# LeeBY68/Hier-SLAM

Measured on AMD Instinct MI355X. Metric: fwd+bwd renders/sec @1200x680, 500k Gaussians, 4-level tree; grad max-abs-err vs ref, higher is better.
Workload: dtype f32; 1 GPU; semantic fwd+bwd render, 1200x680, P=500000 slam Gaussians, K=26 semantic channels, dense upstream grads on colour/semantic/depth/median/opacity; P=500000, visible=480888, num_rendered=1136056, width=1200, height=680, K=26, parallelism=single GPU, keyframes_per_rank=1

## Files before the change

hier-slam_amd/csrc/hsr_render_fwd.hip:

```cpp

#include "hsr_tile_common.h"

#ifdef HSR_TRACE
__device__ unsigned long long g_hsr_trace_fwd[16384 * 8];
extern "C" int hsr_debug_read_trace_fwd(unsigned long long* host, int n)
{
    return (int)hipMemcpyFromSymbol(host, HIP_SYMBOL(g_hsr_trace_fwd), sizeof(unsigned long long) * (size_t)n);
}
#define TRF_NOW() clock64()
#define TRF_ADD(acc, t0) (acc) += (unsigned long long)(clock64() - (t0))
#else
#define TRF_NOW() 0ll
#define TRF_ADD(acc, t0) ((void)0)
#endif

namespace {

template <int W>
__device__ __forceinline__ void quad_fma_words(float (&s)[16], const float (&x)[4], float w)
{
    static_assert(W >= 1 && W <= 4, "1..4 words = 4..16 channels per block");
    if constexpr (W == 4) {
        asm("s_nop 1\n\t"
            "v_fmac_f32_dpp %0, %16, %20 quad_perm:[0,0,0,0] row_mask:0xf bank_mask:0xf\n\t"
            "v_fmac_f32_dpp %1, %16, %20 quad_perm:[1,1,1,1] row_mask:0xf bank_mask:0xf\n\t"
            "v_fmac_f32_dpp %2, %16, %20 quad_perm:[2,2,2,2] row_mask:0xf bank_mask:0xf\n\t"
            "v_fmac_f32_dpp %3, %16, %20 quad_perm:[3,3,3,3] row_mask:0xf bank_mask:0xf\n\t"
            "v_fmac_f32_dpp %4, %17, %20 quad_perm:[0,0,0,0] row_mask:0xf bank_mask:0xf\n\t"
            "v_fmac_f32_dpp %5, %17, %20 quad_perm:[1,1,1,1] row_mask:0xf bank_mask:0xf\n\t"
            "v_fmac_f32_dpp %6, %17, %20 quad_perm:[2,2,2,2] row_mask:0xf bank_mask:0xf\n\t"
            "v_fmac_f32_dpp %7, %17, %20 quad_perm:[3,3,3,3] row_mask:0xf bank_mask:0xf\n\t"
            "v_fmac_f32_dpp %8, %18, %20 quad_perm:[0,0,0,0] row_mask:0xf bank_mask:0xf\n\t"
            "v_fmac_f32_dpp %9, %18, %20 quad_perm:[1,1,1,1] row_mask:0xf bank_mask:0xf\n\t"
            "v_fmac_f32_dpp %10, %18, %20 quad_perm:[2,2,2,2] row_mask:0xf bank_mask:0xf\n\t"
            "v_fmac_f32_dpp %11, %18, %20 quad_perm:[3,3,3,3] row_mask:0xf bank_mask:0xf\n\t"
            "v_fmac_f32_dpp %12, %19, %20 quad_perm:[0,0,0,0] row_mask:0xf bank_mask:0xf\n\t"
            "v_fmac_f32_dpp %13, %19, %20 quad_perm:[1,1,1,1] row_mask:0xf bank_mask:0xf\n\t"
            "v_fmac_f32_dpp %14, %19, %20 quad_perm:[2,2,2,2] row_mask:0xf bank_mask:0xf\n\t"
            "v_fmac_f32_dpp %15, %19, %20 quad_perm:[3,3,3,3] row_mask:0xf bank_mask:0xf"
            : "+v"(s[0]), "+v"(s[1]), "+v"(s[2]), "+v"(s[3]), "+v"(s[4]), "+v"(s[5]), "+v"(s[6]), "+v"(s[7]), "+v"(s[8]), "+v"(s[9]), "+v"(s[10]), "+v"(s[11]), "+v"(s[12]), "+v"(s[13]), "+v"(s[14]), "+v"(s[15])
            : "v"(x[0]), "v"(x[1]), "v"(x[2]), "v"(x[3]), "v"(w));
    } else if constexpr (W == 3) {
        asm("s_nop 1\n\t"
            "v_fmac_f32_dpp %0, %12, %15 quad_perm:[0,0,0,0] row_mask:0xf bank_mask:0xf\n\t"
            "v_fmac_f32_dpp %1, %12, %15 quad_perm:[1,1,1,1] row_mask:0xf bank_mask:0xf\n\t"
            "v_fmac_f32_dpp %2, %12, %15 quad_perm:[2,2,2,2] row_mask:0xf bank_mask:0xf\n\t"
            "v_fmac_f32_dpp %3, %12, %15 quad_perm:[3,3,3,3] row_mask:0xf bank_mask:0xf\n\t"
            "v_fmac_f32_dpp %4, %13, %15 quad_perm:[0,0,0,0] row_mask:0xf bank_mask:0xf\n\t"
            "v_fmac_f32_dpp %5, %13, %15 quad_perm:[1,1,1,1] row_mask:0xf bank_mask:0xf\n\t"
            "v_fmac_f32_dpp %6, %13, %15 quad_perm:[2,2,2,2] row_mask:0xf bank_mask:0xf\n\t"
            "v_fmac_f32_dpp %7, %13, %15 quad_perm:[3,3,3,3] row_mask:0xf bank_mask:0xf\n\t"
            "v_fmac_f32_dpp %8, %14, %15 quad_perm:[0,0,0,0] row_mask:0xf bank_mask:0xf\n\t"
            "v_fmac_f32_dpp %9, %14, %15 quad_perm:[1,1,1,1] row_mask:0xf bank_mask:0xf\n\t"
            "v_fmac_f32_dpp %10, %14, %15 quad_perm:[2,2,2,2] row_mask:0xf bank_mask:0xf\n\t"
            "v_fmac_f32_dpp %11, %14, %15 quad_perm:[3,3,3,3] row_mask:0xf bank_mask:0xf"
            : "+v"(s[0]), "+v"(s[1]), "+v"(s[2]), "+v"(s[3]), "+v"(s[4]), "+v"(s[5]), "+v"(s[6]), "+v"(s[7]), "+v"(s[8]), "+v"(s[9]), "+v"(s[10]), "+v"(s[11])
            : "v"(x[0]), "v"(x[1]), "v"(x[2]), "v"(w));
    } else if constexpr (W == 2) {
        asm("s_nop 1\n\t"
            "v_fmac_f32_dpp %0, %8, %10 quad_perm:[0,0,0,0] row_mask:0xf bank_mask:0xf\n\t"
            "v_fmac_f32_dpp %1, %8, %10 quad_perm:[1,1,1,1] row_mask:0xf bank_mask:0xf\n\t"
            "v_fmac_f32_dpp %2, %8, %10 quad_perm:[2,2,2,2] row_mask:0xf bank_mask:0xf\n\t"
            "v_fmac_f32_dpp %3, %8, %10 quad_perm:[3,3,3,3] row_mask:0xf bank_mask:0xf\n\t"
            "v_fmac_f32_dpp %4, %9, %10 quad_perm:[0,0,0,0] row_mask:0xf bank_mask:0xf\n\t"
            "v_fmac_f32_dpp %5, %9, %10 quad_perm:[1,1,1,1] row_mask:0xf bank_mask:0xf\n\t"
            "v_fmac_f32_dpp %6, %9, %10 quad_perm:[2,2,2,2] row_mask:0xf bank_mask:0xf\n\t"
            "v_fmac_f32_dpp %7, %9, %10 quad_perm:[3,3,3,3] row_mask:0xf bank_mask:0xf"
            : "+v"(s[0]), "+v"(s[1]), "+v"(s[2]), "+v"(s[3]), "+v"(s[4]), "+v"(s[5]), "+v"(s[6]), "+v"(s[7])
            : "v"(x[0]), "v"(x[1]), "v"(w));
    } else {
        asm("s_nop 1\n\t"
            "v_fmac_f32_dpp %0, %4, %5 quad_perm:[0,0,0,0] row_mask:0xf bank_mask:0xf\n\t"
            "v_fmac_f32_dpp %1, %4, %5 quad_perm:[1,1,1,1] row_mask:0xf bank_mask:0xf\n\t"
            "v_fmac_f32_dpp %2, %4, %5 quad_perm:[2,2,2,2] row_mask:0xf bank_mask:0xf\n\t"
            "v_fmac_f32_dpp %3, %4, %5 quad_perm:[3,3,3,3] row_mask:0xf bank_mask:0xf"
            : "+v"(s[0]), "+v"(s[1]), "+v"(s[2]), "+v"(s[3])
            : "v"(x[0]), "v"(w));
    }
}

template <int KC, bool BASE, bool MASK, bool ALIGNED, bool PF = false>
__global__ void __launch_bounds__(256, KC <= 26 ? (KC == 16 ? 5 : 4) : (PF ? (KC <= 48 ? 4 : (KC <= 80 ? 3 : 2)) : 1)) render_fwd_kernel(RenderFwdArgs a, int c0)
{
    constexpr int BATCH = KC <= 32 ? (KC > 26 ? 200 : 240)
                                   : (KC <= 48 ? 152 : ((KC <= 64 || KC == 74) ? 144 : (KC <= 80 ? 136 : (KC <= 112 ? 144 : 128))));
    static_assert(KC <= 32 || PF, "batch sizes beyond 32 channels assume the touched rows (PF)");
    constexpr int RW = (KC + 2 + 3) & ~3;
    constexpr bool QS = PF && KC > 0;
    constexpr int NGF = QS ? RW / 16 : 0;
    constexpr int REM = QS ? (RW % 16) / 4 : 0;
    __shared__ float4 s_rec[BATCH * 2];
    __shared__ float4 s_row[BATCH * (RW / 4)];
    __shared__ uint8_t s_sublist[16 * HSR_SUB_LSTRIDE];
    __shared__ uint8_t s_subcnt[4][16];
    __shared__ int s_wdone[4];

    const int tile = hsr_block_tile(blockIdx.x, hsr_num_tiles(a.W, a.H));
    if (tile >= hsr_num_tiles(a.W, a.H)) return;
    const int t = threadIdx.x, wv = t >> 6;
    if (a.bin.base) {
        BinState bs;
        if (!hsr_bin_resolve(a.bin, *a.bin.R_dev, &bs)) {
            hsr_poison_tile(a, tile, t, BASE, c0, KC);
            return;
        }
        a.point_list = bs.vals;
        a.masks = bs.vals_unsorted;
    }
    const TileGeom tg = tile_geom_sub(tile, a.W, a.H, t);
    const bool inside = tg.inside;
    const size_t N = (size_t)a.W * a.H;
    float pfx = tg.pfx, pfy = tg.pfy;
    asm volatile("" : "+v"(pfx), "+v"(pfy));
    const float tile_x0 = (float)(tg.tx * HSR_TILE_X), tile_y0 = (float)(tg.ty * HSR_TILE_Y);

    unsigned long long tr_bar = 0, tr_stage = 0, tr_blend = 0, tr_iters = 0, tr_pub = 0;
    (void)tr_pub;
    const long long tr_t0 = TRF_NOW();
    long long tr_t1 = tr_t0;
    (void)tr_bar; (void)tr_stage; (void)tr_blend; (void)tr_iters; (void)tr_t0; (void)tr_t1;
    const uint2 range = a.ranges[tile];
    const int n = (int)(range.y - range.x);

    float T = 1.0f;
    uint32_t last_contributor = 0;
    float C0 = 0, C1 = 0, C2 = 0, Dd = 0, Mm = 0;
    uint32_t median_at = 0;
    float median_D = 15.0f;
    float S[KC > 0 ? KC : 1];
#pragma unroll
    for (int c = 0; c < (KC > 0 ? KC : 1); c++) S[c] = 0.f;
    bool done = !inside;

    int id_next = 0;
    float2 p_xy = {0, 0};
    float4 p_co = {0, 0, 0, 0};
    float p_r = 0, p_g = 0, p_b = 0, p_d = 0;
    float p_sem[(KC > 0 && !PF) ? KC : 1];
#pragma unroll
    for (int c = 0; c < ((KC > 0 && !PF) ? KC : 1); c++) p_sem[c] = 0.f;
    constexpr int NPF = PF ? (KC + 15) / 16 + 1 : 1;
    float pf_t[NPF];
#pragma unroll
    for (int c = 0; c < NPF; c++) pf_t[c] = 0.f;
    float pf_sink = 0.f;
    int id_cur = 0;

    auto fetch_id = [&](int start) -> int { return (int)a.point_list[range.x + min(max(start + t, 0), n - 1)]; };
    auto load_record = [&](int id_of) {
        const size_t id = (size_t)id_of;
        id_cur = id_of;
        {
            const float4* rec = a.rec + 4 * id;
            const float4 r0 = rec[0];
            p_co = rec[1];
            p_xy = make_float2(r0.x, r0.y);
            p_d = r0.z;
            if (BASE) {
                const float4 r2 = rec[2];
                p_r = r2.x; p_g = r2.y; p_b = r2.z;
            }
            if (KC > 0 && PF) {
                const float* row = a.semantics + id * (size_t)a.K + c0;
                const int last = min(KC, a.K - c0) - 1;
#pragma unroll
                for (int c = 0; c < NPF; c++) pf_t[c] = row[min(16 * c, last)];
            } else if (KC > 0) {
                if (ALIGNED) {
                    const float2* row = reinterpret_cast<const float2*>(a.semantics + id * (size_t)KC);
#pragma unroll
                    for (int q = 0; q < KC / 2; q++) {
                        const float2 v = row[q];
                        p_sem[PF ? 0 : 2 * q] = v.x;
                        p_sem[PF ? 0 : 2 * q + 1] = v.y;
                    }
                } else {
                    const float* row = a.semantics + id * (size_t)a.K + c0;
#pragma unroll
                    for (int c = 0; c < KC; c++) p_sem[PF ? 0 : c] = (c0 + c < a.K) ? row[c] : 0.f;
                }
            }
        }
    };
    if (n > 0) {
        const int id0 = fetch_id(0);
        id_next = fetch_id(BATCH);
        load_record(id0);
    }
    auto resolve_median = [&](int start) {
        if (BASE && median_at > (uint32_t)start) {
            const int j = (int)median_at - 1 - start;
            constexpr int c = KC + 1;
            constexpr int pos = (QS && c / 16 < NGF) ? (16 * (c / 16) + 4 * (c % 4) + (c % 16) / 4) : c;
            median_D = reinterpret_cast<const float*>(s_row)[j * RW + pos];
        }
    };


    for (int start = 0; start < n; start += BATCH) {
        const bool wave_done = __ballot(!done) == 0ull;
        if ((t & 63) == 0) s_wdone[wv] = wave_done;
        const long long tb0 = TRF_NOW();
        (void)tb0;
        __syncthreads();
        TRF_ADD(tr_bar, tb0);
        if (start == 0) tr_t1 = TRF_NOW();
        const long long ts0 = TRF_NOW();
        (void)ts0;
        if (s_wdone[0] & s_wdone[1] & s_wdone[2] & s_wdone[3]) break;
        const int cnt = min(BATCH, n - start);
        uint32_t mask16 = 0u;
        if (t < cnt) {
            mask16 = subblock_mask(p_xy.x, p_xy.y, p_co.x, p_co.y, p_co.z, p_co.w, tile_x0, tile_y0);
            a.masks[range.x + start + t] = mask16;
            s_rec[2 * t] = make_float4(p_xy.x, p_xy.y, (-0.5f * HSR_LOG2E) * p_co.x, -HSR_LOG2E * p_co.y);
            s_rec[2 * t + 1] = make_float4((-0.5f * HSR_LOG2E) * p_co.z, p_co.w, p_r, p_g);
            float4* row = &s_row[t * (RW / 4)];
            if (PF) {
#pragma unroll
                for (int c = 0; c < NPF; c++) pf_sink += pf_t[c];
                const float* grow = a.semantics + (size_t)id_cur * (size_t)a.K + c0;
                if (mask16 != 0u || t == 0)
#pragma unroll
                for (int g0 = 0; g0 < RW; g0 += 32) {
                    float rv[32];
#pragma unroll
                    for (int c = 0; c < 32; c++) {
                        const int ch = g0 + c;
                        if (ch < KC) {
                            if (ALIGNED) {
                                if ((c & 1) == 0) {
                                    const float2 v = reinterpret_cast<const float2*>(grow)[ch / 2];
                                    rv[c] = v.x;
                                    if (c + 1 < 32) rv[c + 1] = v.y;
                                }
                            } else {
                                rv[c] = (c0 + ch < a.K) ? grow[ch] : 0.f;
                            }
                        } else if (ch < RW) {
                            rv[c] = ch == KC ? p_b : (ch == KC + 1 ? p_d : 0.f);
                        }
                    }
#pragma unroll
                    for (int q = 0; q < 8; q++)
                        if (g0 / 4 + q < RW / 4) {
                            if (QS && g0 / 16 + q / 4 < NGF) {
                                const int b = 16 * (q / 4) + (q & 3);
                                row[g0 / 4 + q] = make_float4(rv[b], rv[b + 4], rv[b + 8], rv[b + 12]);
                            } else {
                                row[g0 / 4 + q] = make_float4(rv[4 * q], rv[4 * q + 1], rv[4 * q + 2], rv[4 * q + 3]);
                            }
                        }
                    asm volatile("" ::: "memory");
                }
            } else {
                float rv[RW];
#pragma unroll
                for (int c = 0; c < RW; c++) rv[c] = c < KC ? p_sem[(c < KC && !PF) ? c : 0] : (c == KC ? p_b : (c == KC + 1 ? p_d : 0.f));
#pragma unroll
                for (int q = 0; q < RW / 4; q++) {
                    if (QS && q / 4 < NGF) {
                        const int b = 16 * (q / 4) + (q & 3);
                        row[q] = make_float4(rv[b], rv[b + 4], rv[b + 8], rv[b + 12]);
                    } else {
                        row[q] = make_float4(rv[4 * q], rv[4 * q + 1], rv[4 * q + 2], rv[4 * q + 3]);
                    }
                }
            }
        }
        const long long tp0 = TRF_NOW();
        (void)tp0;
        publish_subblock_lists(mask16, t, s_sublist, s_subcnt);
        TRF_ADD(tr_pub, tp0);
        TRF_ADD(tr_stage, ts0);
        const long long tb1 = TRF_NOW();
        (void)tb1;
        __syncthreads();
        TRF_ADD(tr_bar, tb1);
        const long long tl0 = TRF_NOW();
        (void)tl0;
        {
            const int id_use = id_next;
            id_next = fetch_id(start + 2 * BATCH);
            load_record(id_use);
        }
        if (wave_done) continue;

        const int lane = t & 63, sb = wv * 4 + (lane >> 4);
        const int total = flatten_sublist(sb, lane, s_sublist, s_subcnt);
        const int m = __builtin_amdgcn_readfirstlane(max(max(__builtin_amdgcn_readlane(total, 0), __builtin_amdgcn_readlane(total, 16)),
                                                         max(__builtin_amdgcn_readlane(total, 32), __builtin_amdgcn_readlane(total, 48))));
        const uint8_t* list = s_sublist + sb * HSR_SUB_LSTRIDE;
        if (total == 0 && (lane & 15) == 0) s_sublist[sb * HSR_SUB_LSTRIDE] = 0;
        __builtin_amdgcn_fence(__ATOMIC_RELEASE, "wavefront");
        __builtin_amdgcn_wave_barrier();
        __builtin_amdgcn_fence(__ATOMIC_ACQUIRE, "wavefront");
        const int last = max(total - 1, 0);
        if constexpr (QS) {
            constexpr int NW = 4 * NGF + REM;
            constexpr int NCH = KC + (BASE ? 2 : 0);
            int j_next = (int)list[0];
            for (int k = 0; k < m; k++) {
                const int j = j_next;
                const bool valid = k < total;
                j_next = (int)list[min(k + 1, last)];
                const float4 g = s_rec[2 * j];
                const float4 h4 = s_rec[2 * j + 1];
                const float2 co = make_float2(h4.x, h4.y);
                const float dx = g.x - pfx, dy = g.y - pfy;
                const float power2 = fmaf(co.x, dy * dy, fmaf(g.w, dx * dy, g.z * (dx * dx)));
                const float alpha = fminf(0.99f, co.y * __builtin_amdgcn_exp2f(power2));
                bool contrib = valid && !done && power2 <= 0.0f && alpha >= 1.0f / 255.0f;
                const float test_T = T * (1.0f - alpha);
                if (contrib && test_T < 0.0001f) {
                    done = true;
                    contrib = false;
                }
                if (__ballot(contrib) == 0ull) continue;
                const float w = contrib ? alpha * T : 0.f;
                if (BASE) {
                    C0 = fmaf(h4.z, w, C0);
                    C1 = fmaf(h4.w, w, C1);
                    if (MASK) Mm += w;
                }
                const float* rowf = reinterpret_cast<const float*>(s_row) + j * RW;
                float fq[NW];
#pragma unroll
                for (int G = 0; G < NGF; G++) {
                    const float4 f = *reinterpret_cast<const float4*>(rowf + 16 * G + 4 * (lane & 3));
                    fq[4 * G] = f.x; fq[4 * G + 1] = f.y; fq[4 * G + 2] = f.z; fq[4 * G + 3] = f.w;
                }
#pragma unroll
                for (int mm = 0; mm < REM; mm++) fq[4 * NGF + mm] = rowf[16 * NGF + 4 * mm + (lane & 3)];
                float dummy = 0.f;
                auto acc = [&](int c) -> float& { return c < KC ? S[c < KC ? c : 0] : ((BASE && c == KC) ? C2 : ((BASE && c == KC + 1) ? Dd : dummy)); };
#pragma unroll
                for (int b = 0; b < (NCH + 15) / 16; b++) {
                    const int nw = min(4, (NCH - 16 * b + 3) / 4);
                    float sv[16], xv[4];
#pragma unroll
                    for (int i = 0; i < 16; i++) sv[i] = i < 4 * nw ? acc(16 * b + i) : 0.f;
#pragma unroll
                    for (int i = 0; i < 4; i++) xv[i] = i < nw ? fq[4 * b + i] : 0.f;
                    if (nw == 4) quad_fma_words<4>(sv, xv, w);
                    else if (nw == 3) quad_fma_words<3>(sv, xv, w);
                    else if (nw == 2) quad_fma_words<2>(sv, xv, w);
                    else quad_fma_words<1>(sv, xv, w);
#pragma unroll
                    for (int i = 0; i < 16; i++)
                        if (i < 4 * nw && 16 * b + i < NCH) acc(16 * b + i) = sv[i];
                }
                if (BASE) {
                    if (contrib && T > 0.5f && test_T < 0.5f) median_at = (uint32_t)(start + j + 1);
                }
                if (contrib) {
                    T = test_T;
                    last_contributor = (uint32_t)(start + j + 1);
                }
#ifdef HSR_TRACE
                tr_iters++;
#endif
            }
        } else {
            int j_next = (int)list[0];
            for (int k = 0; k < m; k++) {
                const int j = j_next;
                const bool valid = k < total;
                j_next = (int)list[min(k + 1, last)];
                const float4 g = s_rec[2 * j];
                const float4 h4 = s_rec[2 * j + 1];
                const float2 co = make_float2(h4.x, h4.y);
                const float dx = g.x - pfx, dy = g.y - pfy;
                const float power2 = fmaf(co.x, dy * dy, fmaf(g.w, dx * dy, g.z * (dx * dx)));
                const float alpha = fminf(0.99f, co.y * __builtin_amdgcn_exp2f(power2));
                bool contrib = valid && !done && power2 <= 0.0f && alpha >= 1.0f / 255.0f;
                const float test_T = T * (1.0f - alpha);
                if (contrib && test_T < 0.0001f) {
                    done = true;
                    contrib = false;
                }
                if (__ballot(contrib) == 0ull) continue;
                const float w = contrib ? alpha * T : 0.f;
                if (BASE) {
                    C0 = fmaf(h4.z, w, C0);
                    C1 = fmaf(h4.w, w, C1);
                    if (MASK) Mm += w;
                }
                {
                    const float4* row = &s_row[j * (RW / 4)];
#pragma unroll
                    for (int q = 0; q < RW / 4; q++) {
                        const float4 f = row[q];
                        const float fv[4] = {f.x, f.y, f.z, f.w};
#pragma unroll
                        for (int i = 0; i < 4; i++) {
                            const int c = 4 * q + i;
                            if (c < KC) S[c < KC ? c : 0] = fmaf(fv[i], w, S[c < KC ? c : 0]);
                            else if (BASE && c == KC) C2 = fmaf(fv[i], w, C2);
                            else if (BASE && c == KC + 1) {
                                Dd = fmaf(fv[i], w, Dd);
                                if (contrib && T > 0.5f && test_T < 0.5f) median_at = (uint32_t)(start + j + 1);
                            }
                        }
                    }
                }
                if (contrib) {
                    T = test_T;
                    last_contributor = (uint32_t)(start + j + 1);
                }
#ifdef HSR_TRACE
                tr_iters++;
#endif
            }
        }
        TRF_ADD(tr_blend, tl0);
        resolve_median(start);
        continue;
    }

    if (PF && pf_sink == 1.2345678e-30f) T = pf_sink;
#ifdef HSR_TRACE
    const long long tr_t2 = clock64();
#endif
    if (inside) {
        const size_t pix_id = (size_t)a.W * (size_t)(int)pfy + (size_t)(int)pfx;
        if (BASE) {
            a.final_T[pix_id] = T;
            a.n_contrib[pix_id] = last_contributor;
            a.median_pos[pix_id] = median_at;
            a.out_color[pix_id] = C0;
            a.out_color[N + pix_id] = C1;
            a.out_color[2 * N + pix_id] = C2;
            a.out_depth[pix_id] = Dd;
            a.out_median_depth[pix_id] = median_D;
            a.out_opacity[pix_id] = 1.0f - T;
            if (MASK) a.out_mask[pix_id] = Mm;
        }
        if (KC > 0) {
#pragma unroll
            for (int c = 0; c < KC; c++)
                if (c0 + c < a.K) a.out_semantic[(size_t)(c0 + c) * N + pix_id] = S[c];
        }
    }
#ifdef HSR_TRACE
    if ((t & 63) == 0) {
        const int wid = tile * 4 + wv;
        if (wid < 16384) {
            unsigned long long* o = g_hsr_trace_fwd + (size_t)wid * 8;
            o[0] = (unsigned long long)(clock64() - tr_t0);
            o[1] = (unsigned long long)(tr_t1 - tr_t0);
            o[2] = tr_bar; o[3] = tr_stage; o[4] = tr_blend;
            o[5] = (unsigned long long)(clock64() - tr_t2);
            o[6] = tr_iters;
            o[7] = tr_pub;
        }
    }
#endif
}

}

int hsr_launch_render_forward(const RenderFwdArgs& a, hipStream_t stream)
{
    const dim3 grid(hsr_tile_grid(hsr_num_tiles(a.W, a.H))), block(256);
    if (!a.semantic) {
        render_fwd_kernel<0, true, true, false><<<grid, block, 0, stream>>>(a, 0);
        return HSR_OK;
    }
    if (a.K >= 27 && a.K <= 128 && a.K != 74 && a.K != 102) {
        if (a.K <= 32) render_fwd_kernel<32, true, false, false, true><<<grid, block, 0, stream>>>(a, 0);
        else if (a.K <= 48) render_fwd_kernel<48, true, false, false, true><<<grid, block, 0, stream>>>(a, 0);
        else if (a.K <= 64) render_fwd_kernel<64, true, false, false, true><<<grid, block, 0, stream>>>(a, 0);
        else if (a.K <= 80) render_fwd_kernel<80, true, false, false, true><<<grid, block, 0, stream>>>(a, 0);
        else if (a.K <= 96) render_fwd_kernel<96, true, false, false, true><<<grid, block, 0, stream>>>(a, 0);
        else if (a.K <= 112) render_fwd_kernel<112, true, false, false, true><<<grid, block, 0, stream>>>(a, 0);
        else render_fwd_kernel<128, true, false, false, true><<<grid, block, 0, stream>>>(a, 0);
        return HSR_OK;
    }
    switch (a.K) {
    case 0: render_fwd_kernel<0, true, false, false><<<grid, block, 0, stream>>>(a, 0); return HSR_OK;
    case 16: render_fwd_kernel<16, true, false, true><<<grid, block, 0, stream>>>(a, 0); return HSR_OK;
    case 26: render_fwd_kernel<26, true, false, true><<<grid, block, 0, stream>>>(a, 0); return HSR_OK;
    case 74: render_fwd_kernel<74, true, false, true, true><<<grid, block, 0, stream>>>(a, 0); return HSR_OK;
    case 102: render_fwd_kernel<102, true, false, true, true><<<grid, block, 0, stream>>>(a, 0); return HSR_OK;
    default:
        render_fwd_kernel<32, true, false, false><<<grid, block, 0, stream>>>(a, 0);
        for (int c0 = 32; c0 < a.K; c0 += 32) render_fwd_kernel<32, false, false, false><<<grid, block, 0, stream>>>(a, c0);
        return HSR_OK;
    }
}
```

hier-slam_amd/csrc/hsr_tile_common.h:

```cpp
#pragma once
#include "hsr_common.h"

#define HSR_LOG2E 1.4426950408889634f

__host__ __device__ inline int hsr_num_tiles(int W, int H) { return ((W + HSR_TILE_X - 1) / HSR_TILE_X) * ((H + HSR_TILE_Y - 1) / HSR_TILE_Y); }
__host__ __device__ inline int hsr_tile_grid(int T) { return 8 * ((T + 7) / 8); }
__device__ __forceinline__ int hsr_block_tile(int b, int T) { return (b & 7) * ((T + 7) >> 3) + (b >> 3); }

__device__ __forceinline__ void hsr_poison_tile(const RenderFwdArgs& a, int tile, int t, bool base, int c0, int nsem)
{
    const int tiles_x = (a.W + HSR_TILE_X - 1) / HSR_TILE_X;
    const int px = (tile % tiles_x) * HSR_TILE_X + (t & 15), py = (tile / tiles_x) * HSR_TILE_Y + (t >> 4);
    if (px >= a.W || py >= a.H) return;
    const size_t N = (size_t)a.W * a.H, pix = (size_t)a.W * py + px;
    const float nan = __uint_as_float(0x7fc00000u);
    if (base) {
        a.out_color[pix] = nan; a.out_color[N + pix] = nan; a.out_color[2 * N + pix] = nan;
        a.out_depth[pix] = nan; a.out_median_depth[pix] = nan; a.out_opacity[pix] = nan;
        if (a.out_mask) a.out_mask[pix] = nan;
    }
    if (a.out_semantic)
        for (int c = c0; c < c0 + nsem && c < a.K; c++) a.out_semantic[(size_t)c * N + pix] = nan;
}

struct TileGeom {
    int tx, ty;
    int px, py;
    bool inside;
    float pfx, pfy;
    float qx0, qy0;
};

__device__ __forceinline__ TileGeom tile_geom(int tile, int W, int H, int t)
{
    TileGeom g;
    const int tiles_x = (W + HSR_TILE_X - 1) / HSR_TILE_X;
    g.tx = tile % tiles_x;
    g.ty = tile / tiles_x;
    const int wv = t >> 6, l = t & 63;
    const int qx = (wv & 1) * 8, qy = (wv >> 1) * 8;
    g.px = g.tx * HSR_TILE_X + qx + (l & 7);
    g.py = g.ty * HSR_TILE_Y + qy + (l >> 3);
    g.inside = g.px < W && g.py < H;
    g.pfx = (float)g.px;
    g.pfy = (float)g.py;
    g.qx0 = (float)(g.tx * HSR_TILE_X + qx);
    g.qy0 = (float)(g.ty * HSR_TILE_Y + qy);
    return g;
}

__device__ __forceinline__ void publish_quadrant_lists(uint32_t qmask, int t, uint8_t (*s_list)[256], uint8_t (*s_lcnt)[4])
{
    const int lane = t & 63, sw = t >> 6;
    const uint64_t lt = (1ull << lane) - 1ull;
#pragma unroll
    for (int q = 0; q < 4; q++) {
        const bool on = (qmask >> q) & 1u;
        const uint64_t m = __ballot(on);
        if (on) s_list[q][sw * 64 + __popcll(m & lt)] = (uint8_t)t;
        if (lane == 0) s_lcnt[q][sw] = (uint8_t)__popcll(m);
    }
}

__device__ __forceinline__ int build_flat_list(int wv, int lane, const uint8_t (*s_list)[256], const uint8_t (*s_lcnt)[4],
                                               uint8_t (*s_flat)[256])
{
    int total = 0;
#pragma unroll
    for (int seg = 0; seg < 4; seg++) {
        const int c = s_lcnt[wv][seg];
        if (lane < c) s_flat[wv][total + lane] = s_list[wv][seg * 64 + lane];
        total += c;
    }
    __builtin_amdgcn_wave_barrier();
    return total;
}

__device__ __forceinline__ TileGeom tile_geom_sub(int tile, int W, int H, int t)
{
    TileGeom g;
    const int tiles_x = (W + HSR_TILE_X - 1) / HSR_TILE_X;
    g.tx = tile % tiles_x;
    g.ty = tile / tiles_x;
    const int wv = t >> 6, l = t & 63, gq = l >> 4;
    const int qx = (wv & 1) * 8 + (gq & 1) * 4, qy = (wv >> 1) * 8 + (gq >> 1) * 4;
    g.px = g.tx * HSR_TILE_X + qx + (l & 3);
    g.py = g.ty * HSR_TILE_Y + qy + ((l >> 2) & 3);
    g.inside = g.px < W && g.py < H;
    g.pfx = (float)g.px;
    g.pfy = (float)g.py;
    g.qx0 = (float)(g.tx * HSR_TILE_X + qx);
    g.qy0 = (float)(g.ty * HSR_TILE_Y + qy);
    return g;
}

__device__ __forceinline__ uint32_t subblock_mask(float x, float y, float cx, float cy, float cz, float opacity, float tile_x0,
                                                  float tile_y0)
{
    const float t255 = 255.0f * opacity;
    if (!(t255 >= 1.0f)) return 0u;
    const float tau = 2.0f * __logf(t255) * 1.002f + 0.02f;
    const float det = cx * cz - cy * cy;
    if (!(det > 0.0f) || !(cx > 0.0f) || !(cz > 0.0f)) return 0xFFFFu;
    const float inv_det = 1.0f / det, inv_a = 1.0f / cx;
    const float hx = sqrtf(tau * cz * inv_det), hy = sqrtf(tau * cx * inv_det) * 1.001f + 0.02f;
    const float dyp = -(cy / cz) * hx;
    const float atau = cx * tau, nb = -cy;
    const float rx = x - tile_x0, ry = y - tile_y0;
    uint32_t m = 0u;
    float ry_hi = ry;
#pragma nounroll
    for (int r = 0; r < 4; r++, ry_hi -= 4.0f) {
        const float lo = fmaxf(ry_hi - 3.0f, -hy), hi = fminf(ry_hi, hy);
        const float dyu = __builtin_amdgcn_fmed3f(dyp, lo, hi), dyl = __builtin_amdgcn_fmed3f(-dyp, lo, hi);
        const float xmax = fmaf(nb, dyu, sqrtf(fmaxf(fmaf(-det * dyu, dyu, atau), 0.0f))) * inv_a + 0.02f;
        const float xmin = fmaf(nb, dyl, -sqrtf(fmaxf(fmaf(-det * dyl, dyl, atau), 0.0f))) * inv_a - 0.02f;
        uint32_t rb = 0u;
#pragma unroll
        for (int c = 0; c < 4; c++)
            rb |= (uint32_t)((rx - (4.0f * c + 3.0f)) <= xmax && (rx - 4.0f * c) >= xmin) << (4 * (c >> 1) + (c & 1));
        if (lo <= hi) m |= rb << (8 * (r >> 1) + 2 * (r & 1));
    }
    return m;
}

__device__ __forceinline__ uint32_t quadrant_bits(uint32_t mask)
{
    return (uint32_t)((mask & 0xFu) != 0u) | ((uint32_t)((mask & 0xF0u) != 0u) << 1) | ((uint32_t)((mask & 0xF00u) != 0u) << 2) |
           ((uint32_t)((mask & 0xF000u) != 0u) << 3);
}
__device__ __forceinline__ uint32_t quadrant_mask_exact(float x, float y, float cx, float cy, float cz, float opacity, float tile_x0,
                                                        float tile_y0)
{
    return quadrant_bits(subblock_mask(x, y, cx, cy, cz, opacity, tile_x0, tile_y0));
}

constexpr int HSR_SUB_LSTRIDE = 260;

__device__ __forceinline__ void publish_subblock_lists(uint32_t mask, int t, uint8_t* s_list, uint8_t (*s_lcnt)[16])
{
    const int lane = t & 63, sw = t >> 6;
    const uint64_t lt = (1ull << lane) - 1ull;
#pragma unroll
    for (int b = 0; b < 16; b++) {
        const bool on = (mask >> b) & 1u;
        const uint64_t m = __ballot(on);
        if (on) s_list[b * HSR_SUB_LSTRIDE + sw * 64 + __popcll(m & lt)] = (uint8_t)t;
        if (lane == 0) s_lcnt[sw][b] = (uint8_t)__popcll(m);
    }
}

__device__ __forceinline__ int flatten_sublist(int sb, int lane, uint8_t* s_list, const uint8_t (*s_lcnt)[16])
{
    const int l16 = lane & 15;
    uint8_t* list = s_list + sb * HSR_SUB_LSTRIDE;
    int total = s_lcnt[0][sb];
#pragma unroll
    for (int seg = 1; seg < 4; seg++) {
        const int c = s_lcnt[seg][sb];
        if (total != seg * 64) {
#pragma unroll
            for (int i = 0; i < 64; i += 16) {
                const bool mv = i + l16 < c;
                const uint8_t v = list[seg * 64 + i + l16];
                if (mv) list[total + i + l16] = v;
            }
        }
        total += c;
    }
    __builtin_amdgcn_wave_barrier();
    return total;
}

#define HSR_GROW_SEM0 16
__host__ __device__ inline int hsr_grow_stride(int K) { return 16 + 16 * ((K + 5 + 15) / 16); }
__host__ __device__ inline int hsr_grow_direct0(int K) { return HSR_GROW_SEM0 + K; }
__host__ __device__ inline int hsr_grow_nl0(int K) { return K + 5 < 9 ? K + 5 : 9; }
__host__ __device__ inline int hsr_grow_stride_l(int layout, int K)
{
    if (!layout) return hsr_grow_stride(K);
    const int R = K + 5 - hsr_grow_nl0(K);
    return 16 + 16 * ((R + 15) / 16);
}
__host__ __device__ inline int hsr_grow_col(int layout, int K, int ch)
{
    if (!layout) return HSR_GROW_SEM0 + ch;
    const int R = K + 5 - hsr_grow_nl0(K);
    return ch < R ? HSR_GROW_SEM0 + ch : 7 + (ch - R);
}
__host__ __device__ inline bool hsr_grow_compact_pays(int K) { return hsr_grow_stride_l(1, K) < hsr_grow_stride(K); }
```

Before: 1820 renders/s.

## Pad sub-block lists with a zero dummy slot to drop per-step bounds checks

For the non-prefetch forward path, each sub-block list is padded up to the wave-max length with an index pointing at a zeroed dummy record slot, so the blend loop no longer clamps indices or tests validity. Termination is folded into T itself (T set to zero on saturation or outside pixels), and a separate T_out keeps the true transmittance for output. Last-contributor and median indices are tracked as batch-relative integers and resolved once per batch rather than per step. This shortens the inner loop and removes branches, at the cost of an extra shared-memory slot, padding writes, and more delicate numerical bookkeeping for early termination.

```diff
diff --git a/hier-slam_amd/csrc/hsr_render_fwd.hip b/hier-slam_amd/csrc/hsr_render_fwd.hip
--- a/hier-slam_amd/csrc/hsr_render_fwd.hip
+++ b/hier-slam_amd/csrc/hsr_render_fwd.hip
@@ -89,8 +89,10 @@
     constexpr bool QS = PF && KC > 0;
     constexpr int NGF = QS ? RW / 16 : 0;
     constexpr int REM = QS ? (RW % 16) / 4 : 0;
-    __shared__ float4 s_rec[BATCH * 2];
-    __shared__ float4 s_row[BATCH * (RW / 4)];
+    constexpr int NSLOT = BATCH + (QS ? 0 : 1);
+    static_assert(NSLOT <= 256, "list entries are bytes");
+    __shared__ float4 s_rec[NSLOT * 2];
+    __shared__ float4 s_row[NSLOT * (RW / 4)];
     __shared__ uint8_t s_sublist[16 * HSR_SUB_LSTRIDE];
     __shared__ uint8_t s_subcnt[4][16];
     __shared__ int s_wdone[4];
@@ -122,7 +124,7 @@
     const uint2 range = a.ranges[tile];
     const int n = (int)(range.y - range.x);
 
-    float T = 1.0f;
+    float T = (QS || inside) ? 1.0f : 0.0f, T_out = 1.0f;
     uint32_t last_contributor = 0;
     float C0 = 0, C1 = 0, C2 = 0, Dd = 0, Mm = 0;
     uint32_t median_at = 0;
@@ -145,6 +147,11 @@
     for (int c = 0; c < NPF; c++) pf_t[c] = 0.f;
     float pf_sink = 0.f;
     int id_cur = 0;
+
+    if constexpr (!QS) {
+        if (t < 2) s_rec[2 * BATCH + t] = make_float4(0.f, 0.f, 0.f, 0.f);
+        if (t < RW / 4) s_row[BATCH * (RW / 4) + t] = make_float4(0.f, 0.f, 0.f, 0.f);
+    }
 
     auto fetch_id = [&](int start) -> int { return (int)a.point_list[range.x + min(max(start + t, 0), n - 1)]; };
     auto load_record = [&](int id_of) {
@@ -198,7 +205,7 @@
 
 
     for (int start = 0; start < n; start += BATCH) {
-        const bool wave_done = __ballot(!done) == 0ull;
+        const bool wave_done = __ballot(QS ? !done : T != 0.0f) == 0ull;
         if ((t & 63) == 0) s_wdone[wv] = wave_done;
         const long long tb0 = TRF_NOW();
         (void)tb0;
@@ -291,12 +298,16 @@
         const int m = __builtin_amdgcn_readfirstlane(max(max(__builtin_amdgcn_readlane(total, 0), __builtin_amdgcn_readlane(total, 16)),
                                                          max(__builtin_amdgcn_readlane(total, 32), __builtin_amdgcn_readlane(total, 48))));
         const uint8_t* list = s_sublist + sb * HSR_SUB_LSTRIDE;
-        if (total == 0 && (lane & 15) == 0) s_sublist[sb * HSR_SUB_LSTRIDE] = 0;
+        if constexpr (QS) {
+            if (total == 0 && (lane & 15) == 0) s_sublist[sb * HSR_SUB_LSTRIDE] = 0;
+        } else {
+            pad_sublist(sb, lane, s_sublist, total, m, BATCH);
+        }
         __builtin_amdgcn_fence(__ATOMIC_RELEASE, "wavefront");
         __builtin_amdgcn_wave_barrier();
         __builtin_amdgcn_fence(__ATOMIC_ACQUIRE, "wavefront");
-        const int last = max(total - 1, 0);
         if constexpr (QS) {
+            const int last = max(total - 1, 0);
             constexpr int NW = 4 * NGF + REM;
             constexpr int NCH = KC + (BASE ? 2 : 0);
             int j_next = (int)list[0];
@@ -362,25 +373,27 @@
 #endif
             }
         } else {
-            int j_next = (int)list[0];
+            const int base1 = start + 1;
+            int last_rel = (int)last_contributor - base1, med_rel = (int)median_at - base1;
+            int j = (int)list[0];
             for (int k = 0; k < m; k++) {
-                const int j = j_next;
-                const bool valid = k < total;
-                j_next = (int)list[min(k + 1, last)];
+                const int j_next = (int)list[k + 1];
                 const float4 g = s_rec[2 * j];
                 const float4 h4 = s_rec[2 * j + 1];
                 const float2 co = make_float2(h4.x, h4.y);
                 const float dx = g.x - pfx, dy = g.y - pfy;
                 const float power2 = fmaf(co.x, dy * dy, fmaf(g.w, dx * dy, g.z * (dx * dx)));
                 const float alpha = fminf(0.99f, co.y * __builtin_amdgcn_exp2f(power2));
-                bool contrib = valid && !done && power2 <= 0.0f && alpha >= 1.0f / 255.0f;
+                const bool reach = power2 <= 0.0f && alpha >= 1.0f / 255.0f;
                 const float test_T = T * (1.0f - alpha);
-                if (contrib && test_T < 0.0001f) {
-                    done = true;
-                    contrib = false;
-                }
-                if (__ballot(contrib) == 0ull) continue;
+                const bool low = test_T < 0.0001f;
+                const bool contrib = reach && !low;
                 const float w = contrib ? alpha * T : 0.f;
+                if (__ballot(contrib) == 0ull) {
+                    T = reach ? 0.0f : T;
+                    j = j_next;
+                    continue;
+                }
                 if (BASE) {
                     C0 = fmaf(h4.z, w, C0);
                     C1 = fmaf(h4.w, w, C1);
@@ -397,24 +410,26 @@
                             const int c = 4 * q + i;
                             if (c < KC) S[c < KC ? c : 0] = fmaf(fv[i], w, S[c < KC ? c : 0]);
                             else if (BASE && c == KC) C2 = fmaf(fv[i], w, C2);
-                            else if (BASE && c == KC + 1) {
-                                Dd = fmaf(fv[i], w, Dd);
-                                if (contrib && T > 0.5f && test_T < 0.5f) median_at = (uint32_t)(start + j + 1);
-                            }
+                            else if (BASE && c == KC + 1) Dd = fmaf(fv[i], w, Dd);
                         }
                     }
                 }
-                if (contrib) {
-                    T = test_T;
-                    last_contributor = (uint32_t)(start + j + 1);
-                }
+                const float T_was = T_out;
+                T_out = contrib ? test_T : T_out;
+                if (BASE) med_rel = (T_was > 0.5f && T_out < 0.5f) ? j : med_rel;
+                last_rel = contrib ? j : last_rel;
+                T = reach ? (low ? 0.0f : test_T) : T;
+                j = j_next;
 #ifdef HSR_TRACE
                 tr_iters++;
 #endif
             }
+            last_contributor = (uint32_t)(last_rel + base1);
+            median_at = (uint32_t)(med_rel + base1);
+            if (BASE && med_rel >= 0) median_D = reinterpret_cast<const float*>(s_row)[med_rel * RW + KC + 1];
         }
         TRF_ADD(tr_blend, tl0);
-        resolve_median(start);
+        if constexpr (QS) resolve_median(start);
         continue;
     }
 
@@ -425,7 +440,8 @@
     if (inside) {
         const size_t pix_id = (size_t)a.W * (size_t)(int)pfy + (size_t)(int)pfx;
         if (BASE) {
-            a.final_T[pix_id] = T;
+            const float T_fin = QS ? T : T_out;
+            a.final_T[pix_id] = T_fin;
             a.n_contrib[pix_id] = last_contributor;
             a.median_pos[pix_id] = median_at;
             a.out_color[pix_id] = C0;
@@ -433,7 +449,7 @@
             a.out_color[2 * N + pix_id] = C2;
             a.out_depth[pix_id] = Dd;
             a.out_median_depth[pix_id] = median_D;
-            a.out_opacity[pix_id] = 1.0f - T;
+            a.out_opacity[pix_id] = 1.0f - T_fin;
             if (MASK) a.out_mask[pix_id] = Mm;
         }
         if (KC > 0) {
diff --git a/hier-slam_amd/csrc/hsr_tile_common.h b/hier-slam_amd/csrc/hsr_tile_common.h
--- a/hier-slam_amd/csrc/hsr_tile_common.h
+++ b/hier-slam_amd/csrc/hsr_tile_common.h
@@ -172,6 +172,12 @@
     return total;
 }
 
+__device__ __forceinline__ void pad_sublist(int sb, int lane, uint8_t* s_list, int total, int m, int dummy)
+{
+    uint8_t* list = s_list + sb * HSR_SUB_LSTRIDE;
+    for (int p = total + (lane & 15); p <= m; p += 16) list[p] = (uint8_t)dummy;
+}
+
 #define HSR_GROW_SEM0 16
 __host__ __device__ inline int hsr_grow_stride(int K) { return 16 + 16 * ((K + 5 + 15) / 16); }
 __host__ __device__ inline int hsr_grow_direct0(int K) { return HSR_GROW_SEM0 + K; }
```

New measurement: 1844 renders/s (median of 6 runs). +1.3%, better.
